# ANRGUSC/DEFER

Hardware: NVIDIA H100
Metric: inferences_per_sec (higher is better)
Workload: dtype bf16x3->f32

## Files before the change

defer_b200/csrc/conv_umma.cu:

```cuda
#include <cuda.h>
#include <string.h>

#include <type_traits>

#include <vector>

#include "common.cuh"
#include "conv_umma.cuh"

namespace defer {

static int env_int(const char* name, int dflt) {
  const char* v = getenv(name);
  return v ? atoi(v) : dflt;
}

namespace {

constexpr int BM = 128;
constexpr int BK = 64;
constexpr int CONS_THREADS = 256;
constexpr int NUM_THREADS = CONS_THREADS + 128;
constexpr int SMEM_CAP = 227 * 1024 - 256;
constexpr int CTL_BYTES = 256;
constexpr int MAX_STAGES = 8;
constexpr int MEGA_BN = 64;
constexpr int STG_COLS = 64;
constexpr int STG_BYTES = BM * STG_COLS * 4;

struct KParams {
  int n, ho, wo, cout;
  int tile_h, tile_w, tiles_h, tiles_w;
  int im2col;
  int m_total;
  int kh, kw, sh, sw, pad_t, pad_l;
  int cblocks;
  int k_blocks;
  int splits;
  int cluster;
  uint32_t flags;
  const float* scale;
  const float* shift;
  const void* res;
  void* y;
  float* partial;
  unsigned int* counters;
  size_t plane_out;
};

struct alignas(128) MegaOp {
  CUtensorMap tmx[2];
  CUtensorMap tmw[2];
  KParams p;
  int m_tiles, n_tiles;
  const float* stem_x;
  int stem_h, stem_w, stem_cin, stem_kh, stem_kw, stem_sh, stem_sw, stem_pad_t, stem_pad_l, stem_K;
  int stem_win_rows, stem_win_cols;
  const uint8_t* stem_u8;
  float stem_shift[3];
  const float* scale2;
  const float* shift2;
  void* y2;
  int relu2;
  int store_first;
};

template <int NPLANES, int BN>
struct Smem {
  static constexpr int A_PLANE = BM * 128;
  static constexpr int B_PLANE = BN * 128;
  static constexpr int STAGE = NPLANES * (A_PLANE + B_PLANE);
  static constexpr int RED = BM * BN * 4;
  __host__ __device__ static constexpr int ring(int stages, bool red) {
    return (red && stages * STAGE < RED) ? RED : stages * STAGE;
  }
  __host__ __device__ static constexpr int total(int stages, bool red) {
    return ring(stages, red) + STG_BYTES + CTL_BYTES + 1024;
  }
  __host__ __device__ static constexpr int max_stages() {
    return (SMEM_CAP - STG_BYTES - CTL_BYTES - 1024) / STAGE > MAX_STAGES ? MAX_STAGES
                                                                          : (SMEM_CAP - STG_BYTES - CTL_BYTES - 1024) / STAGE;
  }
};
static_assert(Smem<2, 128>::max_stages() == 3 && Smem<2, 64>::max_stages() == 4, "BF16X2 ring depths");
static_assert(Smem<1, 64>::max_stages() == 8 && Smem<1, 128>::max_stages() == 6, "BF16 ring depths");

__device__ __forceinline__ uint32_t smem_u32(const void* p) { return (uint32_t)__cvta_generic_to_shared(p); }

__device__ __forceinline__ void mbar_init(uint32_t bar, uint32_t count) {
  asm volatile("mbarrier.init.shared::cta.b64 [%0], %1;" ::"r"(bar), "r"(count));
}
__device__ __forceinline__ void mbar_arrive_expect_tx(uint32_t bar, uint32_t bytes) {
  asm volatile("mbarrier.arrive.expect_tx.shared::cta.b64 _, [%0], %1;" ::"r"(bar), "r"(bytes) : "memory");
}
__device__ __forceinline__ void mbar_expect_tx(uint32_t bar, uint32_t bytes) {
  asm volatile("mbarrier.expect_tx.relaxed.cta.shared::cta.b64 [%0], %1;" ::"r"(bar), "r"(bytes) : "memory");
}
__device__ __forceinline__ void mbar_arrive(uint32_t bar) {
  asm volatile("mbarrier.arrive.shared::cta.b64 _, [%0];" ::"r"(bar) : "memory");
}
__device__ __forceinline__ bool mbar_try_wait(uint32_t bar, uint32_t parity) {
  uint32_t ok;
  asm volatile(
      "{\n.reg .pred p;\n"
      "mbarrier.try_wait.parity.shared::cta.b64 p, [%1], %2;\n"
      "selp.u32 %0, 1, 0, p;\n}\n"
      : "=r"(ok)
      : "r"(bar), "r"(parity)
      : "memory");
  return ok != 0;
}
__device__ __forceinline__ unsigned long long gtimer() {
  unsigned long long t;
  asm volatile("mov.u64 %0, %%globaltimer;" : "=l"(t));
  return t;
}
__device__ int g_conv_wait_timeout_tag;
__device__ __forceinline__ void mbar_wait(uint32_t bar, uint32_t parity, int tag) {
  if (mbar_try_wait(bar, parity)) return;
  unsigned long long t0 = gtimer();
  unsigned spins = 0;
  while (!mbar_try_wait(bar, parity)) {
    if ((++spins & 0xfff) == 0 && gtimer() - t0 > 2000000000ull) {
      g_conv_wait_timeout_tag = tag;
      asm volatile("trap;");
    }
  }
}

__device__ __forceinline__ void tma_load_4d(uint32_t dst, const CUtensorMap* map, uint32_t bar, int c0, int c1, int c2,
                                            int c3) {
  asm volatile(
      "cp.async.bulk.tensor.4d.shared::cluster.global.mbarrier::complete_tx::bytes [%0], [%1, {%3, %4, %5, %6}], [%2];"
      ::"r"(dst), "l"(reinterpret_cast<uint64_t>(map)), "r"(bar), "r"(c0), "r"(c1), "r"(c2), "r"(c3)
      : "memory");
}
__device__ __forceinline__ void tma_load_im2col_4d(uint32_t dst, const CUtensorMap* map, uint32_t bar, int c0, int w, int h,
                                                   int n, uint16_t ow, uint16_t oh) {
  asm volatile(
      "cp.async.bulk.tensor.4d.shared::cluster.global.im2col.mbarrier::complete_tx::bytes [%0], [%1, {%3, %4, %5, %6}], "
      "[%2], {%7, %8};"
      ::"r"(dst), "l"(reinterpret_cast<uint64_t>(map)), "r"(bar), "r"(c0), "r"(w), "r"(h), "r"(n), "h"(ow), "h"(oh)
      : "memory");
}
__device__ __forceinline__ void tma_load_3d(uint32_t dst, const CUtensorMap* map, uint32_t bar, int c0, int c1, int c2) {
  asm volatile(
      "cp.async.bulk.tensor.3d.shared::cluster.global.mbarrier::complete_tx::bytes [%0], [%1, {%3, %4, %5}], [%2];"
      ::"r"(dst), "l"(reinterpret_cast<uint64_t>(map)), "r"(bar), "r"(c0), "r"(c1), "r"(c2)
      : "memory");
}

__device__ __forceinline__ void cluster_sync_all() {
  asm volatile("barrier.cluster.arrive.release.aligned;" ::: "memory");
  asm volatile("barrier.cluster.wait.acquire.aligned;" ::: "memory");
}
__device__ __forceinline__ uint32_t cluster_ctarank() {
  uint32_t r;
  asm volatile("mov.u32 %0, %%cluster_ctarank;" : "=r"(r));
  return r;
}
__device__ __forceinline__ uint32_t cluster_nctarank() {
  uint32_t r;
  asm volatile("mov.u32 %0, %%cluster_nctarank;" : "=r"(r));
  return r;
}
__device__ __forceinline__ uint32_t dsmem_map(uint32_t local_addr, uint32_t rank) {
  uint32_t r;
  asm volatile("mapa.shared::cluster.u32 %0, %1, %2;" : "=r"(r) : "r"(local_addr), "r"(rank));
  return r;
}
__device__ __forceinline__ float4 dsmem_ld4(uint32_t addr) {
  float4 v;
  asm volatile("ld.shared::cluster.v4.f32 {%0, %1, %2, %3}, [%4];" : "=f"(v.x), "=f"(v.y), "=f"(v.z), "=f"(v.w) : "r"(addr));
  return v;
}
__device__ __forceinline__ void cons_bar_sync() { asm volatile("bar.sync 1, 256;" ::: "memory"); }
__device__ __forceinline__ void prod_bar_sync() { asm volatile("bar.sync 2, 128;" ::: "memory"); }

__device__ __forceinline__ uint64_t make_sw128_desc(uint32_t smem_addr) {
  return (uint64_t)((smem_addr & 0x3FFFF) >> 4) | (1ull << 16) | (64ull << 32) | (1ull << 62);
}
__device__ __forceinline__ void wg_fence() { asm volatile("wgmma.fence.sync.aligned;" ::: "memory"); }
__device__ __forceinline__ void wg_commit() { asm volatile("wgmma.commit_group.sync.aligned;" ::: "memory"); }
template <int N>
__device__ __forceinline__ void wg_wait() {
  asm volatile("wgmma.wait_group.sync.aligned %0;" ::"n"(N) : "memory");
}
template <int R>
__device__ __forceinline__ void acc_fence(float (&d)[R]) {
#pragma unroll
  for (int i = 0; i < R; ++i) asm volatile("" : "+f"(d[i])::"memory");
}

template <int BN>
__device__ __forceinline__ void wgmma_bf16(float (&d)[BN / 2], uint64_t a, uint64_t b);

template <>
__device__ __forceinline__ void wgmma_bf16<64>(float (&d)[32], uint64_t a, uint64_t b) {
  asm volatile(
      "{\n.reg .pred p;\nsetp.ne.b32 p, %34, 0;\n"
      "wgmma.mma_async.sync.aligned.m64n64k16.f32.bf16.bf16 "
      "{%0, %1, %2, %3, %4, %5, %6, %7, %8, %9, %10, %11, %12, %13, %14, %15, %16, %17, %18, %19, %20, %21, %22, "
      "%23, %24, %25, %26, %27, %28, %29, %30, %31}, %32, %33, p, 1, 1, 0, 0;\n}\n"
      : "+f"(d[0]), "+f"(d[1]), "+f"(d[2]), "+f"(d[3]), "+f"(d[4]), "+f"(d[5]), "+f"(d[6]), "+f"(d[7]), "+f"(d[8]),
        "+f"(d[9]), "+f"(d[10]), "+f"(d[11]), "+f"(d[12]), "+f"(d[13]), "+f"(d[14]), "+f"(d[15]), "+f"(d[16]),
        "+f"(d[17]), "+f"(d[18]), "+f"(d[19]), "+f"(d[20]), "+f"(d[21]), "+f"(d[22]), "+f"(d[23]), "+f"(d[24]),
        "+f"(d[25]), "+f"(d[26]), "+f"(d[27]), "+f"(d[28]), "+f"(d[29]), "+f"(d[30]), "+f"(d[31])
      : "l"(a), "l"(b), "r"(1));
}

template <>
__device__ __forceinline__ void wgmma_bf16<128>(float (&d)[64], uint64_t a, uint64_t b) {
  asm volatile(
      "{\n.reg .pred p;\nsetp.ne.b32 p, %66, 0;\n"
      "wgmma.mma_async.sync.aligned.m64n128k16.f32.bf16.bf16 "
      "{%0, %1, %2, %3, %4, %5, %6, %7, %8, %9, %10, %11, %12, %13, %14, %15, %16, %17, %18, %19, %20, %21, %22, "
      "%23, %24, %25, %26, %27, %28, %29, %30, %31, %32, %33, %34, %35, %36, %37, %38, %39, %40, %41, %42, %43, %44, "
      "%45, %46, %47, %48, %49, %50, %51, %52, %53, %54, %55, %56, %57, %58, %59, %60, %61, %62, %63}, %64, %65, p, "
      "1, 1, 0, 0;\n}\n"
      : "+f"(d[0]), "+f"(d[1]), "+f"(d[2]), "+f"(d[3]), "+f"(d[4]), "+f"(d[5]), "+f"(d[6]), "+f"(d[7]), "+f"(d[8]),
        "+f"(d[9]), "+f"(d[10]), "+f"(d[11]), "+f"(d[12]), "+f"(d[13]), "+f"(d[14]), "+f"(d[15]), "+f"(d[16]),
        "+f"(d[17]), "+f"(d[18]), "+f"(d[19]), "+f"(d[20]), "+f"(d[21]), "+f"(d[22]), "+f"(d[23]), "+f"(d[24]),
        "+f"(d[25]), "+f"(d[26]), "+f"(d[27]), "+f"(d[28]), "+f"(d[29]), "+f"(d[30]), "+f"(d[31]), "+f"(d[32]),
        "+f"(d[33]), "+f"(d[34]), "+f"(d[35]), "+f"(d[36]), "+f"(d[37]), "+f"(d[38]), "+f"(d[39]), "+f"(d[40]),
        "+f"(d[41]), "+f"(d[42]), "+f"(d[43]), "+f"(d[44]), "+f"(d[45]), "+f"(d[46]), "+f"(d[47]), "+f"(d[48]),
        "+f"(d[49]), "+f"(d[50]), "+f"(d[51]), "+f"(d[52]), "+f"(d[53]), "+f"(d[54]), "+f"(d[55]), "+f"(d[56]),
        "+f"(d[57]), "+f"(d[58]), "+f"(d[59]), "+f"(d[60]), "+f"(d[61]), "+f"(d[62]), "+f"(d[63])
      : "l"(a), "l"(b), "r"(1));
}

template <bool STEM>
__device__ __forceinline__ void row_to_pixel(const KParams& p, int r, int n0, int h0, int w0, bool& valid, size_t& pix) {
  if (!STEM) {
    const int m = w0 + r;
    valid = m < p.m_total;
    pix = (size_t)m;
  } else {
    const int th = r / p.tile_w;
    const int oh = h0 + th, ow = w0 + r % p.tile_w;
    valid = th < p.tile_h && oh < p.ho && ow < p.wo;
    pix = ((size_t)n0 * p.ho + oh) * p.wo + ow;
  }
}

struct EpiArgs {
  const float* scale;
  const float* shift;
  const __nv_bfloat16* res;
  __nv_bfloat16* y;
  size_t plane;
  int cout;
  bool relu;
  bool store_first;
  bool relu2;
  const float* scale2;
  const float* shift2;
  __nv_bfloat16* y2;
};

__device__ __forceinline__ EpiArgs epi_args(const MegaOp& op) {
  const KParams& p = op.p;
  EpiArgs e;
  e.scale = p.scale;
  e.shift = p.shift;
  e.res = reinterpret_cast<const __nv_bfloat16*>(p.res);
  e.y = reinterpret_cast<__nv_bfloat16*>(p.y);
  e.plane = p.plane_out;
  e.cout = p.cout;
  e.relu = (p.flags & DEFER_FLAG_RELU) != 0;
  e.store_first = op.store_first != 0;
  e.relu2 = op.relu2 != 0;
  e.scale2 = op.scale2;
  e.shift2 = op.shift2;
  e.y2 = reinterpret_cast<__nv_bfloat16*>(op.y2);
  return e;
}

__device__ __forceinline__ uint32_t stg_off(int r, int c) {
  return (uint32_t)(r * STG_COLS + (((c >> 2) ^ ((r & 7) << 1)) << 2) + (c & 3)) * 4u;
}
__device__ __forceinline__ void sts2(uint32_t addr, float a, float b) {
  asm volatile("st.shared.v2.f32 [%0], {%1, %2};" ::"r"(addr), "f"(a), "f"(b));
}
__device__ __forceinline__ float4 lds4(uint32_t addr) {
  float4 v;
  asm volatile("ld.shared.v4.f32 {%0, %1, %2, %3}, [%4];" : "=f"(v.x), "=f"(v.y), "=f"(v.z), "=f"(v.w) : "r"(addr));
  return v;
}
__device__ __forceinline__ void stg4(void* p, uint4 v) {
  asm volatile("st.global.v4.b32 [%0], {%1, %2, %3, %4};" ::"l"(p), "r"(v.x), "r"(v.y), "r"(v.z), "r"(v.w));
}

__device__ __forceinline__ float bf_lo(uint32_t w) { return __uint_as_float(w << 16); }
__device__ __forceinline__ float bf_hi(uint32_t w) { return __uint_as_float(w & 0xffff0000u); }

template <int NPLANES, int BN, bool AFF, bool STEM = false>
__device__ __forceinline__ void epi_tile(const KParams& p, const EpiArgs& e, uint32_t stg, const float (&acc)[BN / 2],
                                         uint32_t qmask, int c_base, int n0, int h0, int w0) {
  const int tid = threadIdx.x;
  const int lane = tid & 31;
  const int row0 = (tid >> 7) * 64 + ((tid >> 5) & 3) * 16 + (lane >> 2);
  const int col_l = 2 * (lane & 3);
  const int jg = tid & 7;
  const int rb = tid >> 3;
  const int ca = 2 * jg + ((jg >> 2) & 1), cb = ca ^ 1;
  const bool swap = (jg >> 2) & 1;
  size_t orow[4];
  uint32_t vmask = 0;
#pragma unroll
  for (int k = 0; k < 4; ++k) {
    bool v;
    size_t pix;
    row_to_pixel<STEM>(p, rb + 32 * k, n0, h0, w0, v, pix);
    orow[k] = pix * (size_t)e.cout;
    vmask |= (uint32_t)v << k;
  }
#pragma unroll
  for (int P = 0; P < BN / STG_COLS; ++P) {
    const bool mine = (qmask >> (8 * P + jg)) & 1u;
    const int c = c_base + STG_COLS * P + 8 * jg;
    cons_bar_sync();
#pragma unroll
    for (int qq = 0; qq < 8; ++qq) {
      const int q = 8 * P + qq;
      if (!((qmask >> q) & 1u)) continue;
      sts2(stg + stg_off(row0, 8 * qq + col_l), acc[4 * q], acc[4 * q + 1]);
      sts2(stg + stg_off(row0 + 8, 8 * qq + col_l), acc[4 * q + 2], acc[4 * q + 3]);
    }
    uint4 rh[4], rl[4];
#pragma unroll
    for (int k = 0; k < 4; ++k) {
      rh[k] = rl[k] = make_uint4(0u, 0u, 0u, 0u);
      if (e.res && mine && ((vmask >> k) & 1u)) {
        rh[k] = __ldcg(reinterpret_cast<const uint4*>(e.res + orow[k] + c));
        if (NPLANES == 2) rl[k] = __ldcg(reinterpret_cast<const uint4*>(e.res + e.plane + orow[k] + c));
      }
    }
    float sc[8], sf[8];
#pragma unroll
    for (int i = 0; i < 8; ++i) { sc[i] = 1.f; sf[i] = 0.f; }
    if (mine) {
      if (e.scale) {
        const float4 a = __ldg(reinterpret_cast<const float4*>(e.scale + c));
        const float4 b = __ldg(reinterpret_cast<const float4*>(e.scale + c + 4));
        sc[0] = a.x; sc[1] = a.y; sc[2] = a.z; sc[3] = a.w; sc[4] = b.x; sc[5] = b.y; sc[6] = b.z; sc[7] = b.w;
      }
      if (e.shift) {
        const float4 a = __ldg(reinterpret_cast<const float4*>(e.shift + c));
        const float4 b = __ldg(reinterpret_cast<const float4*>(e.shift + c + 4));
        sf[0] = a.x; sf[1] = a.y; sf[2] = a.z; sf[3] = a.w; sf[4] = b.x; sf[5] = b.y; sf[6] = b.z; sf[7] = b.w;
      }
    }
    cons_bar_sync();
    if (!mine) continue;

#pragma unroll
    for (int k = 0; k < 4; ++k) {
      if (!((vmask >> k) & 1u)) continue;
      const int r = rb + 32 * k;
      const float4 xa = lds4(stg + stg_off(r, 4 * ca));
      const float4 xb = lds4(stg + stg_off(r, 4 * cb));
      const float4 x0 = swap ? xb : xa, x1 = swap ? xa : xb;
      float v[8] = {x0.x, x0.y, x0.z, x0.w, x1.x, x1.y, x1.z, x1.w};
      const uint32_t hw[4] = {rh[k].x, rh[k].y, rh[k].z, rh[k].w};
      const uint32_t lw[4] = {rl[k].x, rl[k].y, rl[k].z, rl[k].w};
#pragma unroll
      for (int i = 0; i < 8; ++i) {
        v[i] = fmaf(v[i], sc[i], sf[i]);
        if (e.res) {
          v[i] += (i & 1) ? bf_hi(hw[i >> 1]) : bf_lo(hw[i >> 1]);
          if (NPLANES == 2) v[i] += (i & 1) ? bf_hi(lw[i >> 1]) : bf_lo(lw[i >> 1]);
        }
        if (e.relu) v[i] = fmaxf(v[i], 0.f);
      }
      uint4 hi, lo = make_uint4(0u, 0u, 0u, 0u);
      if (NPLANES == 2) {
        split_bf16x2(v[0], v[1], hi.x, lo.x);
        split_bf16x2(v[2], v[3], hi.y, lo.y);
        split_bf16x2(v[4], v[5], hi.z, lo.z);
        split_bf16x2(v[6], v[7], hi.w, lo.w);
      } else {
        hi = make_uint4(pack_bf16x2(v[0], v[1]), pack_bf16x2(v[2], v[3]), pack_bf16x2(v[4], v[5]), pack_bf16x2(v[6], v[7]));
      }
      const size_t o = orow[k] + c;
      if (!AFF || e.store_first) {
        stg4(e.y + o, hi);
        if (NPLANES == 2) stg4(e.y + e.plane + o, lo);
      }
      if constexpr (AFF) {
        float s2[8], t2[8];
        {
          const float4 a = __ldg(reinterpret_cast<const float4*>(e.scale2 + c));
          const float4 b = __ldg(reinterpret_cast<const float4*>(e.scale2 + c + 4));
          const float4 d = __ldg(reinterpret_cast<const float4*>(e.shift2 + c));
          const float4 f = __ldg(reinterpret_cast<const float4*>(e.shift2 + c + 4));
          s2[0] = a.x; s2[1] = a.y; s2[2] = a.z; s2[3] = a.w; s2[4] = b.x; s2[5] = b.y; s2[6] = b.z; s2[7] = b.w;
          t2[0] = d.x; t2[1] = d.y; t2[2] = d.z; t2[3] = d.w; t2[4] = f.x; t2[5] = f.y; t2[6] = f.z; t2[7] = f.w;
        }
        const uint32_t sh[4] = {hi.x, hi.y, hi.z, hi.w};
        const uint32_t sl[4] = {lo.x, lo.y, lo.z, lo.w};
        float u[8];
#pragma unroll
        for (int i = 0; i < 8; ++i) {
          u[i] = (i & 1) ? bf_hi(sh[i >> 1]) : bf_lo(sh[i >> 1]);
          if (NPLANES == 2) u[i] = u[i] + ((i & 1) ? bf_hi(sl[i >> 1]) : bf_lo(sl[i >> 1]));
          u[i] = fmaf(u[i], s2[i], t2[i]);
          if (e.relu2) u[i] = fmaxf(u[i], 0.f);
        }
        uint4 h2, l2;
        if (NPLANES == 2) {
          split_bf16x2(u[0], u[1], h2.x, l2.x);
          split_bf16x2(u[2], u[3], h2.y, l2.y);
          split_bf16x2(u[4], u[5], h2.z, l2.z);
          split_bf16x2(u[6], u[7], h2.w, l2.w);
          stg4(e.y2 + o, h2);
          stg4(e.y2 + e.plane + o, l2);
        } else {
          h2 = make_uint4(pack_bf16x2(u[0], u[1]), pack_bf16x2(u[2], u[3]), pack_bf16x2(u[4], u[5]), pack_bf16x2(u[6], u[7]));
          stg4(e.y2 + o, h2);
        }
      }
    }
  }
}

template <int NPLANES, int BN, int MODE, bool AFF = false>
__device__ __forceinline__ void conv_body(const MegaOp* ops, int n_ops, int stages, int pdl) {
  using L = Smem<NPLANES, BN>;
  constexpr int R = BN / 2;
  extern __shared__ uint8_t smem_raw[];
  uint8_t* smem = reinterpret_cast<uint8_t*>((reinterpret_cast<uintptr_t>(smem_raw) + 1023) & ~(uintptr_t)1023);
  const uint32_t ring = smem_u32(smem);
  const bool red = MODE == 0 && ops[0].p.cluster;
  const uint32_t stg = ring + L::ring(stages, red);
  const uint32_t bar_base = stg + STG_BYTES;
  auto full_bar = [&](int s) { return bar_base + 8u * s; };
  auto empty_bar = [&](int s) { return bar_base + 8u * (stages + s); };
  __shared__ int s_is_last;

  const int tid = threadIdx.x;
  if (tid == 0) {
    for (int s = 0; s < stages; ++s) {
      mbar_init(full_bar(s), 1);
      mbar_init(empty_bar(s), CONS_THREADS / 32);
    }
    asm volatile("fence.mbarrier_init.release.cluster;" ::: "memory");
  }
  __syncthreads();
  if (pdl) {
    asm volatile("griddepcontrol.wait;" ::: "memory");
    asm volatile("griddepcontrol.launch_dependents;" ::: "memory");
  }

  uint32_t it = 0;
  for (int o = 0; o < n_ops; ++o) {
    const MegaOp& op = ops[o];
    const KParams& p = op.p;
    const int total = op.m_tiles * op.n_tiles;
    int t_first, t_step;
    if (MODE == 0) {
      t_first = blockIdx.y * op.m_tiles + blockIdx.x;
      t_step = total;
    } else if (MODE == 1) {
      t_first = blockIdx.x;
      t_step = gridDim.x;
    } else {
      t_first = (int)cluster_ctarank();
      t_step = (int)cluster_nctarank();
    }
    const int split = MODE == 0 ? (int)blockIdx.z : 0;
    const int kb_begin = (split * p.k_blocks) / p.splits;
    const int kb_end = ((split + 1) * p.k_blocks) / p.splits;

    for (int t = t_first; t < total; t += t_step) {
      const int m0 = (t % op.m_tiles) * BM;
      const int c_base = (t / op.m_tiles) * BN;

      if (tid >= CONS_THREADS) {
        if (tid == CONS_THREADS) {
          const int ow = m0 % p.wo;
          const int oh = (m0 / p.wo) % p.ho;
          const int cw = ow * p.sw - p.pad_l, ch = oh * p.sh - p.pad_t, cn = m0 / (p.wo * p.ho);
          uint32_t i2 = it;
          for (int kb = kb_begin; kb < kb_end; ++kb, ++i2) {
            const int stage = (int)(i2 % (uint32_t)stages);
            const uint32_t phase = (i2 / (uint32_t)stages) & 1u;
            mbar_wait(empty_bar(stage), phase ^ 1u, 1);
            const uint32_t a_dst = ring + stage * L::STAGE;
            const uint32_t b_dst = a_dst + NPLANES * L::A_PLANE;
            const int tap = kb / p.cblocks;
            const int cb = kb - tap * p.cblocks;
            const uint16_t khi = (uint16_t)(tap / p.kw);
            const uint16_t kwi = (uint16_t)(tap - khi * p.kw);
            mbar_arrive_expect_tx(full_bar(stage), NPLANES * (uint32_t)(L::A_PLANE + L::B_PLANE));
#pragma unroll
            for (int pl = 0; pl < NPLANES; ++pl) {
              if (p.im2col)
                tma_load_im2col_4d(a_dst + pl * L::A_PLANE, &op.tmx[pl], full_bar(stage), cb * BK, cw, ch, cn, kwi, khi);
              else
                tma_load_4d(a_dst + pl * L::A_PLANE, &op.tmx[pl], full_bar(stage), cb * BK, m0, 0, 0);
              tma_load_3d(b_dst + pl * L::B_PLANE, &op.tmw[pl], full_bar(stage), cb * BK, c_base, tap);
            }
          }
        }
        it += (uint32_t)(kb_end - kb_begin);
        continue;
      }

      const int wg = tid >> 7;
      const int lane = tid & 31;
      float acc[R];
#pragma unroll
      for (int i = 0; i < R; ++i) acc[i] = 0.f;
      int prev_stage = -1;
      for (int kb = kb_begin; kb < kb_end; ++kb, ++it) {
        const int stage = (int)(it % (uint32_t)stages);
        mbar_wait(full_bar(stage), (it / (uint32_t)stages) & 1u, 2);
        const uint32_t a_addr = ring + stage * L::STAGE + wg * (64 * 128);
        const uint32_t b_addr = ring + stage * L::STAGE + NPLANES * L::A_PLANE;
        wg_fence();
#pragma unroll
        for (int k = 0; k < BK / 16; ++k) {
          const uint64_t a_hi = make_sw128_desc(a_addr + k * 32);
          const uint64_t b_hi = make_sw128_desc(b_addr + k * 32);
          wgmma_bf16<BN>(acc, a_hi, b_hi);
          if (NPLANES == 2) {
            wgmma_bf16<BN>(acc, make_sw128_desc(a_addr + L::A_PLANE + k * 32), b_hi);
            wgmma_bf16<BN>(acc, a_hi, make_sw128_desc(b_addr + L::B_PLANE + k * 32));
          }
        }
        wg_commit();
        wg_wait<1>();
        acc_fence(acc);
        if (prev_stage >= 0 && lane == 0) mbar_arrive(empty_bar(prev_stage));
        prev_stage = stage;
      }
      wg_wait<0>();
      acc_fence(acc);
      if (prev_stage >= 0 && lane == 0) mbar_arrive(empty_bar(prev_stage));


      if (MODE == 0 && p.cluster) {
        cons_bar_sync();
        float4* red_buf = reinterpret_cast<float4*>(smem);
#pragma unroll
        for (int q = 0; q < R / 4; ++q)
          red_buf[q * CONS_THREADS + tid] = make_float4(acc[4 * q], acc[4 * q + 1], acc[4 * q + 2], acc[4 * q + 3]);
        break;
      }
      if (MODE == 0 && p.splits > 1) {
        const size_t tile_lin = (size_t)t;
        float4* mine = reinterpret_cast<float4*>(p.partial) + (tile_lin * p.splits + split) * (R / 4) * CONS_THREADS;
#pragma unroll
        for (int q = 0; q < R / 4; ++q)
          __stcg(mine + q * CONS_THREADS + tid, make_float4(acc[4 * q], acc[4 * q + 1], acc[4 * q + 2], acc[4 * q + 3]));
        __threadfence();
        cons_bar_sync();
        if (tid == 0) {
          const unsigned prev = atomicAdd(p.counters + tile_lin, 1u);
          const int last = prev == (unsigned)(p.splits - 1);
          if (last) p.counters[tile_lin] = 0;
          s_is_last = last;
        }
        cons_bar_sync();
        if (!s_is_last) continue;
        __threadfence();
#pragma unroll
        for (int i = 0; i < R; ++i) acc[i] = 0.f;
        for (int s = 0; s < p.splits; ++s) {
          const float4* src = reinterpret_cast<const float4*>(p.partial) + (tile_lin * p.splits + s) * (R / 4) * CONS_THREADS;
#pragma unroll
          for (int q = 0; q < R / 4; ++q) {
            const float4 v = __ldcg(src + q * CONS_THREADS + tid);
            acc[4 * q] += v.x; acc[4 * q + 1] += v.y; acc[4 * q + 2] += v.z; acc[4 * q + 3] += v.w;
          }
        }
      }
      epi_tile<NPLANES, BN, AFF>(p, epi_args(op), stg, acc, 0xffffu, c_base, 0, 0, m0);
    }

    if (MODE == 0 && p.cluster) {
      cluster_sync_all();
      if (tid < CONS_THREADS) {
        const int S = p.splits;
        const int rank = (int)cluster_ctarank();
        const uint32_t mine = ring + (uint32_t)tid * 16u;
        float acc[R];
        uint32_t qmask = 0;
#pragma unroll
        for (int q = 0; q < R / 4; ++q) {
          acc[4 * q] = acc[4 * q + 1] = acc[4 * q + 2] = acc[4 * q + 3] = 0.f;
          if (q % S != rank) continue;
          qmask |= 1u << q;
          const uint32_t addr = mine + (uint32_t)(q * CONS_THREADS) * 16u;
          float4 a = dsmem_ld4(dsmem_map(addr, 0));
          for (int s = 1; s < S; ++s) {
            const float4 v = dsmem_ld4(dsmem_map(addr, (uint32_t)s));
            a.x += v.x; a.y += v.y; a.z += v.z; a.w += v.w;
          }
          acc[4 * q] = a.x; acc[4 * q + 1] = a.y; acc[4 * q + 2] = a.z; acc[4 * q + 3] = a.w;
        }
        epi_tile<NPLANES, BN, AFF>(p, epi_args(op), stg, acc, qmask, (int)blockIdx.y * BN, 0, 0, (int)blockIdx.x * BM);
      }
      cluster_sync_all();
    }
    if (MODE == 2 && o + 1 < n_ops) {
      asm volatile("fence.proxy.async.global;" ::: "memory");
      cluster_sync_all();
    }
  }
}

template <int NPLANES, int BN>
__global__ void __launch_bounds__(NUM_THREADS, 1) conv_umma_kernel(const __grid_constant__ MegaOp op, int stages, int pdl) {
  conv_body<NPLANES, BN, 0>(&op, 1, stages, pdl);
}

template <int NPLANES, int BN>
__global__ void __launch_bounds__(NUM_THREADS, 1) conv_stream_kernel(const MegaOp* __restrict__ ops, int stages, int pdl) {
  conv_body<NPLANES, BN, 1>(ops, 1, stages, pdl);
}

template <int NPLANES, int BN>
__global__ void __launch_bounds__(NUM_THREADS, 1) conv_umma_aff_kernel(const __grid_constant__ MegaOp op, int stages, int pdl) {
  conv_body<NPLANES, BN, 0, true>(&op, 1, stages, pdl);
}

template <int NPLANES, int BN>
__global__ void __launch_bounds__(NUM_THREADS, 1) conv_stream_aff_kernel(const MegaOp* __restrict__ ops, int stages, int pdl) {
  conv_body<NPLANES, BN, 1, true>(ops, 1, stages, pdl);
}

template <int NPLANES>
__global__ void __launch_bounds__(NUM_THREADS, 1) conv_mega_kernel(const MegaOp* __restrict__ ops, int n_ops, int stages) {
  conv_body<NPLANES, MEGA_BN, 2>(ops, n_ops, stages, 0);
}

enum StemIn { STEM_F32, STEM_U8_CAFFE, STEM_U8_TF };
constexpr int PROD_THREADS = NUM_THREADS - CONS_THREADS;
constexpr int STEM_WIN_BYTES = 24 * 1024;
constexpr int STEM_WIN_VALS = STEM_WIN_BYTES / 4;
constexpr int STEM_FILL = STEM_WIN_VALS / PROD_THREADS;
constexpr int STEM_TILE_W = 16;

template <int NPLANES>
struct StemSmem {
  static constexpr int STAGE = Smem<NPLANES, 64>::STAGE;
  __host__ __device__ static constexpr int total(int stages) {
    return stages * STAGE + STG_BYTES + 2 * STEM_WIN_BYTES + CTL_BYTES + 1024;
  }
  __host__ __device__ static constexpr int max_stages() {
    return (SMEM_CAP - STG_BYTES - 2 * STEM_WIN_BYTES - CTL_BYTES - 1024) / STAGE > MAX_STAGES
               ? MAX_STAGES
               : (SMEM_CAP - STG_BYTES - 2 * STEM_WIN_BYTES - CTL_BYTES - 1024) / STAGE;
  }
};
static_assert(StemSmem<2>::max_stages() == 3 && StemSmem<1>::max_stages() == 6, "stem ring depths with two image windows");
static_assert(STEM_FILL * PROD_THREADS == STEM_WIN_VALS, "the producer threads cover a whole window");

struct StemGeo {
  const float* x;
  const uint8_t* u8;
  float s0, s1, s2;
  int H, rowlen;
  int cin, sh, sw, pad_t, pad_l;
  int wcols, nwin;
  int run, K;
};

__device__ __forceinline__ StemGeo stem_geo(const MegaOp& op) {
  StemGeo g;
  g.x = op.stem_x;
  g.u8 = op.stem_u8;
  g.s0 = op.stem_shift[0]; g.s1 = op.stem_shift[1]; g.s2 = op.stem_shift[2];
  g.H = op.stem_h;
  g.rowlen = op.stem_w * op.stem_cin;
  g.cin = op.stem_cin; g.sh = op.stem_sh; g.sw = op.stem_sw; g.pad_t = op.stem_pad_t; g.pad_l = op.stem_pad_l;
  g.wcols = op.stem_win_cols;
  g.nwin = op.stem_win_rows * op.stem_win_cols;
  g.run = op.stem_kw * op.stem_cin;
  g.K = op.stem_K;
  return g;
}

__device__ __forceinline__ void stem_tile_origin(const KParams& p, int m_tile, int& n0, int& h0, int& w0) {
  const int t2 = m_tile / p.tiles_w;
  n0 = t2 / p.tiles_h;
  h0 = (t2 - n0 * p.tiles_h) * p.tile_h;
  w0 = (m_tile - t2 * p.tiles_w) * p.tile_w;
}

template <int IN>
__device__ __forceinline__ void stem_fill_load(const StemGeo& g, int ptid, int n0, int h0, int w0, uint32_t (&raw)[STEM_FILL]) {
  const int ih0 = h0 * g.sh - g.pad_t, col0 = (w0 * g.sw - g.pad_l) * g.cin;
  const size_t img = (size_t)n0 * g.H * g.rowlen;
  const int dq = PROD_THREADS / g.wcols, dm = PROD_THREADS - dq * g.wcols;
  int wr = ptid / g.wcols, wc = ptid - wr * g.wcols;
  int c = wc % 3;
#pragma unroll
  for (int j = 0; j < STEM_FILL; ++j) {
    const int ih = ih0 + wr, col = col0 + wc;
    const bool in = ptid + PROD_THREADS * j < g.nwin && ih >= 0 && ih < g.H && col >= 0 && col < g.rowlen;
    const size_t off = img + (size_t)(ih * g.rowlen + col);
    if constexpr (IN == STEM_F32) raw[j] = in ? __float_as_uint(__ldg(g.x + off)) : 0u;
    else raw[j] = in ? (uint32_t)__ldg(g.u8 + off + (IN == STEM_U8_CAFFE ? 2 - 2 * c : 0)) : 0x100u;
    wr += dq;
    wc += dm;
    if (wc >= g.wcols) { wc -= g.wcols; ++wr; }
    c = c == 0 ? 2 : c - 1;
  }
}

template <int IN>
__device__ __forceinline__ void stem_fill_store(const StemGeo& g, uint32_t win, int ptid, const uint32_t (&raw)[STEM_FILL]) {
  int c = (ptid % g.wcols) % 3;
#pragma unroll
  for (int j = 0; j < STEM_FILL; ++j) {
    const int e = ptid + PROD_THREADS * j;
    if (e < g.nwin) {
      const float b = __fsub_rn(__uint_as_float(0x4B000000u | raw[j]), 8388608.f);
      float v;
      if constexpr (IN == STEM_F32) v = __uint_as_float(raw[j]);
      else if constexpr (IN == STEM_U8_CAFFE) v = raw[j] > 255u ? 0.f : __fadd_rn(b, c == 0 ? g.s0 : (c == 1 ? g.s1 : g.s2));
      else v = raw[j] > 255u ? 0.f : keras_tf_preprocess(b);
      asm volatile("st.shared.f32 [%0], %1;" ::"r"(win + 4u * (uint32_t)e), "f"(v) : "memory");
    }
    c = c == 0 ? 2 : c - 1;
  }
}

template <int NPLANES>
__device__ __forceinline__ void stem_build(const StemGeo& g, uint32_t win, uint32_t a_dst, int r, int row_base, int kb) {
  int k = kb * BK;
  int a = k / g.run, jj = k - a * g.run;
  uint32_t src = win + 4u * (uint32_t)(row_base + a * g.wcols + jj);
  const uint32_t wrap = 4u * (uint32_t)(g.wcols - g.run);
#pragma unroll 1
  for (int ch = 0; ch < 8; ++ch) {
    float v[8];
#pragma unroll
    for (int e = 0; e < 8; ++e) {
      v[e] = 0.f;
      if (k < g.K) asm volatile("ld.shared.f32 %0, [%1];" : "=f"(v[e]) : "r"(src));
      ++k;
      src += 4u;
      if (++jj == g.run) { jj = 0; src += wrap; }
    }
    const uint32_t off = (uint32_t)r * 128u + ((uint32_t)(ch ^ (r & 7)) << 4);
    uint32_t h[4], l[4];
#pragma unroll
    for (int q = 0; q < 4; ++q) {
      if (NPLANES == 2) split_bf16x2(v[2 * q], v[2 * q + 1], h[q], l[q]);
      else h[q] = pack_bf16x2(v[2 * q], v[2 * q + 1]);
    }
    asm volatile("st.shared.v4.b32 [%0], {%1, %2, %3, %4};" ::"r"(a_dst + off), "r"(h[0]), "r"(h[1]), "r"(h[2]), "r"(h[3])
                 : "memory");
    if (NPLANES == 2)
      asm volatile("st.shared.v4.b32 [%0], {%1, %2, %3, %4};" ::"r"(a_dst + Smem<NPLANES, 64>::A_PLANE + off), "r"(l[0]),
                   "r"(l[1]), "r"(l[2]), "r"(l[3])
                   : "memory");
  }
}

template <int NPLANES, int IN>
__device__ __forceinline__ void stem_body(const MegaOp* ops, int stages, int pdl) {
  using L = Smem<NPLANES, 64>;
  extern __shared__ uint8_t smem_raw[];
  uint8_t* smem = reinterpret_cast<uint8_t*>((reinterpret_cast<uintptr_t>(smem_raw) + 1023) & ~(uintptr_t)1023);
  const uint32_t ring = smem_u32(smem);
  const uint32_t stg = ring + stages * L::STAGE;
  const uint32_t win0 = stg + STG_BYTES;
  const uint32_t bar_base = win0 + 2 * STEM_WIN_BYTES;
  auto full_bar = [&](int s) { return bar_base + 8u * s; };
  auto empty_bar = [&](int s) { return bar_base + 8u * (stages + s); };

  const int tid = threadIdx.x;
  if (tid == 0) {
    for (int s = 0; s < stages; ++s) {
      mbar_init(full_bar(s), 1);
      mbar_init(empty_bar(s), CONS_THREADS / 32);
    }
    asm volatile("fence.mbarrier_init.release.cluster;" ::: "memory");
  }
  __syncthreads();
  if (pdl) {
    asm volatile("griddepcontrol.wait;" ::: "memory");
    asm volatile("griddepcontrol.launch_dependents;" ::: "memory");
  }

  const MegaOp& op = ops[0];
  const KParams& p = op.p;
  const int total = op.m_tiles * op.n_tiles;
  const int k_blocks = p.k_blocks;
  uint32_t it = 0;

  if (tid >= CONS_THREADS) {
    const int ptid = tid - CONS_THREADS;
    const StemGeo g = stem_geo(op);
    int th = ptid / p.tile_w, tw = ptid - th * p.tile_w;
    if (th >= p.tile_h) th = tw = 0;
    const int row_base = th * g.sh * g.wcols + tw * g.sw * g.cin;
    uint32_t raw[STEM_FILL];
    int n0, h0, w0;
    if ((int)blockIdx.x < total) {
      stem_tile_origin(p, (int)blockIdx.x % op.m_tiles, n0, h0, w0);
      stem_fill_load<IN>(g, ptid, n0, h0, w0, raw);
      stem_fill_store<IN>(g, win0, ptid, raw);
    }
    int wb = 0;
    for (int t = blockIdx.x; t < total; t += gridDim.x, wb ^= 1) {
      const int t_next = t + (int)gridDim.x;
      if (t_next < total) {
        stem_tile_origin(p, t_next % op.m_tiles, n0, h0, w0);
        stem_fill_load<IN>(g, ptid, n0, h0, w0, raw);
      }
      prod_bar_sync();
      const uint32_t win = win0 + (uint32_t)wb * STEM_WIN_BYTES;
      const int c_base = (t / op.m_tiles) * 64;
      for (int kb = 0; kb < k_blocks; ++kb, ++it) {
        const int stage = (int)(it % (uint32_t)stages);
        mbar_wait(empty_bar(stage), ((it / (uint32_t)stages) & 1u) ^ 1u, 1);
        const uint32_t a_dst = ring + stage * L::STAGE;
        const uint32_t b_dst = a_dst + NPLANES * L::A_PLANE;
        if (ptid == 0) {
          mbar_expect_tx(full_bar(stage), NPLANES * (uint32_t)L::B_PLANE);
          tma_load_3d(b_dst, &op.tmw[0], full_bar(stage), kb * BK, c_base, 0);
          if (NPLANES == 2) tma_load_3d(b_dst + L::B_PLANE, &op.tmw[1], full_bar(stage), kb * BK, c_base, 0);
        }
        stem_build<NPLANES>(g, win, a_dst, ptid, row_base, kb);
        asm volatile("fence.proxy.async.shared::cta;" ::: "memory");
        prod_bar_sync();
        if (ptid == 0) mbar_arrive(full_bar(stage));
      }
      if (t_next < total) stem_fill_store<IN>(g, win0 + (uint32_t)(wb ^ 1) * STEM_WIN_BYTES, ptid, raw);
    }
    return;
  }

  const int wg = tid >> 7;
  const int lane = tid & 31;
  for (int t = blockIdx.x; t < total; t += gridDim.x) {
    float acc[32];
#pragma unroll
    for (int i = 0; i < 32; ++i) acc[i] = 0.f;
    int prev_stage = -1;
    for (int kb = 0; kb < k_blocks; ++kb, ++it) {
      const int stage = (int)(it % (uint32_t)stages);
      mbar_wait(full_bar(stage), (it / (uint32_t)stages) & 1u, 2);
      const uint32_t a_addr = ring + stage * L::STAGE + wg * (64 * 128);
      const uint32_t b_addr = ring + stage * L::STAGE + NPLANES * L::A_PLANE;
      wg_fence();
#pragma unroll
      for (int k = 0; k < BK / 16; ++k) {
        const uint64_t a_hi = make_sw128_desc(a_addr + k * 32);
        const uint64_t b_hi = make_sw128_desc(b_addr + k * 32);
        wgmma_bf16<64>(acc, a_hi, b_hi);
        if (NPLANES == 2) {
          wgmma_bf16<64>(acc, make_sw128_desc(a_addr + L::A_PLANE + k * 32), b_hi);
          wgmma_bf16<64>(acc, a_hi, make_sw128_desc(b_addr + L::B_PLANE + k * 32));
        }
      }
      wg_commit();
      wg_wait<1>();
      acc_fence(acc);
      if (prev_stage >= 0 && lane == 0) mbar_arrive(empty_bar(prev_stage));
      prev_stage = stage;
    }
    wg_wait<0>();
    acc_fence(acc);
    if (prev_stage >= 0 && lane == 0) mbar_arrive(empty_bar(prev_stage));
    int n0, h0, w0;
    stem_tile_origin(p, t % op.m_tiles, n0, h0, w0);
    epi_tile<NPLANES, 64, false, true>(p, epi_args(op), stg, acc, 0xffffu, (t / op.m_tiles) * 64, n0, h0, w0);
  }
}

template <int NPLANES>
__global__ void __launch_bounds__(NUM_THREADS, 1) conv_stem_kernel(const MegaOp* __restrict__ ops, int stages, int pdl) {
  stem_body<NPLANES, STEM_F32>(ops, stages, pdl);
}

template <int NPLANES>
__global__ void __launch_bounds__(NUM_THREADS, 1) conv_stem_u8_kernel(const MegaOp* __restrict__ ops, int stages, int pdl) {
  stem_body<NPLANES, STEM_U8_CAFFE>(ops, stages, pdl);
}

template <int NPLANES>
__global__ void __launch_bounds__(NUM_THREADS, 1) conv_stem_u8tf_kernel(const MegaOp* __restrict__ ops, int stages, int pdl) {
  stem_body<NPLANES, STEM_U8_TF>(ops, stages, pdl);
}

__global__ void __launch_bounds__(256) weight_transform_kernel(const float* __restrict__ w, __nv_bfloat16* __restrict__ out,
                                                               int taps, int cin, int cout, int nplanes) {
  size_t total = (size_t)taps * cin * cout;
  size_t i = (size_t)blockIdx.x * blockDim.x + threadIdx.x;
  if (i >= total) return;
  int ci = (int)(i % cin);
  size_t t2 = i / cin;
  int co = (int)(t2 % cout);
  int tap = (int)(t2 / cout);
  float v = w[((size_t)tap * cin + ci) * cout + co];
  __nv_bfloat16 hi = __float2bfloat16_rn(v);
  out[i] = hi;
  if (nplanes == 2) out[total + i] = __float2bfloat16_rn(v - __bfloat162float(hi));
}

typedef CUresult (*PFN_encodeTiled)(CUtensorMap*, CUtensorMapDataType, cuuint32_t, void*, const cuuint64_t*,
                                    const cuuint64_t*, const cuuint32_t*, const cuuint32_t*, CUtensorMapInterleave,
                                    CUtensorMapSwizzle, CUtensorMapL2promotion, CUtensorMapFloatOOBfill);

PFN_encodeTiled get_encode() {
  static PFN_encodeTiled fn = nullptr;
  if (!fn) {
    void* p = nullptr;
    cudaDriverEntryPointQueryResult q;
    if (cudaGetDriverEntryPoint("cuTensorMapEncodeTiled", &p, cudaEnableDefault, &q) == cudaSuccess &&
        q == cudaDriverEntryPointSuccess)
      fn = (PFN_encodeTiled)p;
  }
  return fn;
}

int encode_map(CUtensorMap* map, void* base, int rank, const uint64_t* dims, const uint64_t* strides_bytes,
               const uint32_t* box, const uint32_t* estr) {
  PFN_encodeTiled enc = get_encode();
  if (!enc) {
    set_error("cuTensorMapEncodeTiled entry point not available");
    return DEFER_ERR_CUDA;
  }
  CUresult r = enc(map, CU_TENSOR_MAP_DATA_TYPE_BFLOAT16, (cuuint32_t)rank, base, (const cuuint64_t*)dims,
                   (const cuuint64_t*)strides_bytes, (const cuuint32_t*)box, (const cuuint32_t*)estr,
                   CU_TENSOR_MAP_INTERLEAVE_NONE, CU_TENSOR_MAP_SWIZZLE_128B, CU_TENSOR_MAP_L2_PROMOTION_L2_256B,
                   CU_TENSOR_MAP_FLOAT_OOB_FILL_NONE);
// ... 503 lines not shown
```

Before: 15370.

## Add dedicated warp-specialized stream kernel body with residual prefetch before mainloop

New measurement: 13820 (median of 6 runs). -10.1%, worse.

```diff
diff --git a/defer_b200/csrc/conv_umma.cu b/defer_b200/csrc/conv_umma.cu
--- a/defer_b200/csrc/conv_umma.cu
+++ b/defer_b200/csrc/conv_umma.cu
@@ -294,9 +294,10 @@
 __device__ __forceinline__ float bf_lo(uint32_t w) { return __uint_as_float(w << 16); }
 __device__ __forceinline__ float bf_hi(uint32_t w) { return __uint_as_float(w & 0xffff0000u); }
 
-template <int NPLANES, int BN, bool AFF, bool STEM = false>
+template <int NPLANES, int BN, bool AFF, bool STEM = false, bool PRE = false>
 __device__ __forceinline__ void epi_tile(const KParams& p, const EpiArgs& e, uint32_t stg, const float (&acc)[BN / 2],
-                                         uint32_t qmask, int c_base, int n0, int h0, int w0) {
+                                         uint32_t qmask, int c_base, int n0, int h0, int w0,
+                                         const uint4 (*pre)[2][4] = nullptr) {
   const int tid = threadIdx.x;
   const int lane = tid & 31;
   const int row0 = (tid >> 7) * 64 + ((tid >> 5) & 3) * 16 + (lane >> 2);
@@ -330,6 +331,11 @@
     uint4 rh[4], rl[4];
 #pragma unroll
     for (int k = 0; k < 4; ++k) {
+      if constexpr (PRE) {
+        rh[k] = pre[P][0][k];
+        rl[k] = pre[P][1][k];
+        continue;
+      }
       rh[k] = rl[k] = make_uint4(0u, 0u, 0u, 0u);
       if (e.res && mine && ((vmask >> k) & 1u)) {
         rh[k] = __ldcg(reinterpret_cast<const uint4*>(e.res + orow[k] + c));
@@ -424,6 +430,27 @@
   }
 }
 
+template <int NPLANES, int BN>
+__device__ __forceinline__ void epi_res_prefetch(const KParams& p, const EpiArgs& e, int c_base, int m0,
+                                                 uint4 (&pre)[BN / STG_COLS][2][4]) {
+  const int tid = threadIdx.x;
+  const int c = c_base + 8 * (tid & 7);
+  const int rb = tid >> 3;
+#pragma unroll
+  for (int P = 0; P < BN / STG_COLS; ++P) {
+#pragma unroll
+    for (int k = 0; k < 4; ++k) {
+      const int m = m0 + rb + 32 * k;
+      pre[P][0][k] = pre[P][1][k] = make_uint4(0u, 0u, 0u, 0u);
+      if (e.res && m < p.m_total) {
+        const size_t o = (size_t)m * (size_t)e.cout + (size_t)(c + STG_COLS * P);
+        pre[P][0][k] = __ldcg(reinterpret_cast<const uint4*>(e.res + o));
+        if (NPLANES == 2) pre[P][1][k] = __ldcg(reinterpret_cast<const uint4*>(e.res + e.plane + o));
+      }
+    }
+  }
+}
+
 template <int NPLANES, int BN, int MODE, bool AFF = false>
 __device__ __forceinline__ void conv_body(const MegaOp* ops, int n_ops, int stages, int pdl) {
   using L = Smem<NPLANES, BN>;
@@ -461,9 +488,6 @@
     if (MODE == 0) {
       t_first = blockIdx.y * op.m_tiles + blockIdx.x;
       t_step = total;
-    } else if (MODE == 1) {
-      t_first = blockIdx.x;
-      t_step = gridDim.x;
     } else {
       t_first = (int)cluster_ctarank();
       t_step = (int)cluster_nctarank();
@@ -611,6 +635,115 @@
   }
 }
 
+template <int NPLANES, int BN, bool AFF>
+__device__ __forceinline__ void stream_body(const MegaOp* ops, int stages, int pdl) {
+  using L = Smem<NPLANES, BN>;
+  constexpr int R = BN / 2;
+  extern __shared__ uint8_t smem_raw[];
+  uint8_t* smem = reinterpret_cast<uint8_t*>((reinterpret_cast<uintptr_t>(smem_raw) + 1023) & ~(uintptr_t)1023);
+  const uint32_t ring = smem_u32(smem);
+  const uint32_t stg = ring + L::ring(stages, false);
+  const uint32_t bar_base = stg + STG_BYTES;
+  auto full_bar = [&](int s) { return bar_base + 8u * s; };
+  auto empty_bar = [&](int s) { return bar_base + 8u * (stages + s); };
+
+  const int tid = threadIdx.x;
+  if (tid == 0) {
+    for (int s = 0; s < stages; ++s) {
+      mbar_init(full_bar(s), 1);
+      mbar_init(empty_bar(s), CONS_THREADS / 32);
+    }
+    asm volatile("fence.mbarrier_init.release.cluster;" ::: "memory");
+  }
+  __syncthreads();
+  if (pdl) {
+    asm volatile("griddepcontrol.wait;" ::: "memory");
+    asm volatile("griddepcontrol.launch_dependents;" ::: "memory");
+  }
+
+  const MegaOp& op = ops[0];
+  const KParams& p = op.p;
+
+  if (tid >= CONS_THREADS) {
+    asm volatile("setmaxnreg.dec.sync.aligned.u32 40;" ::: "memory");
+    if (tid != CONS_THREADS) return;
+    const int total = op.m_tiles * op.n_tiles;
+    const int k_blocks = p.k_blocks;
+    uint32_t it = 0;
+    for (int t = blockIdx.x; t < total; t += gridDim.x) {
+      const int m0 = (t % op.m_tiles) * BM;
+      const int c_base = (t / op.m_tiles) * BN;
+      const int ow = m0 % p.wo;
+      const int oh = (m0 / p.wo) % p.ho;
+      const int cw = ow * p.sw - p.pad_l, ch = oh * p.sh - p.pad_t, cn = m0 / (p.wo * p.ho);
+      for (int kb = 0; kb < k_blocks; ++kb, ++it) {
+        const int stage = (int)(it % (uint32_t)stages);
+        mbar_wait(empty_bar(stage), ((it / (uint32_t)stages) & 1u) ^ 1u, 1);
+        const uint32_t a_dst = ring + stage * L::STAGE;
+        const uint32_t b_dst = a_dst + NPLANES * L::A_PLANE;
+        const int tap = kb / p.cblocks;
+        const int cb = kb - tap * p.cblocks;
+        const uint16_t khi = (uint16_t)(tap / p.kw);
+        const uint16_t kwi = (uint16_t)(tap - khi * p.kw);
+        mbar_arrive_expect_tx(full_bar(stage), NPLANES * (uint32_t)(L::A_PLANE + L::B_PLANE));
+#pragma unroll
+        for (int pl = 0; pl < NPLANES; ++pl) {
+          if (p.im2col)
+            tma_load_im2col_4d(a_dst + pl * L::A_PLANE, &op.tmx[pl], full_bar(stage), cb * BK, cw, ch, cn, kwi, khi);
+          else
+            tma_load_4d(a_dst + pl * L::A_PLANE, &op.tmx[pl], full_bar(stage), cb * BK, m0, 0, 0);
+          tma_load_3d(b_dst + pl * L::B_PLANE, &op.tmw[pl], full_bar(stage), cb * BK, c_base, tap);
+        }
+      }
+    }
+    return;
+  }
+
+  asm volatile("setmaxnreg.inc.sync.aligned.u32 232;" ::: "memory");
+  const int total = op.m_tiles * op.n_tiles;
+  const int k_blocks = p.k_blocks;
+  const int wg = tid >> 7;
+  const int lane = tid & 31;
+  uint32_t it = 0;
+  for (int t = blockIdx.x; t < total; t += gridDim.x) {
+    const int m0 = (t % op.m_tiles) * BM;
+    const int c_base = (t / op.m_tiles) * BN;
+    uint4 pre[BN / STG_COLS][2][4];
+    epi_res_prefetch<NPLANES, BN>(p, epi_args(op), c_base, m0, pre);
+
+    float acc[R];
+#pragma unroll
+    for (int i = 0; i < R; ++i) acc[i] = 0.f;
+    int prev_stage = -1;
+    for (int kb = 0; kb < k_blocks; ++kb, ++it) {
+      const int stage = (int)(it % (uint32_t)stages);
+      mbar_wait(full_bar(stage), (it / (uint32_t)stages) & 1u, 2);
+      const uint32_t a_addr = ring + stage * L::STAGE + wg * (64 * 128);
+      const uint32_t b_addr = ring + stage * L::STAGE + NPLANES * L::A_PLANE;
+      wg_fence();
+#pragma unroll
+      for (int k = 0; k < BK / 16; ++k) {
+        const uint64_t a_hi = make_sw128_desc(a_addr + k * 32);
+        const uint64_t b_hi = make_sw128_desc(b_addr + k * 32);
+        wgmma_bf16<BN>(acc, a_hi, b_hi);
+        if (NPLANES == 2) {
+          wgmma_bf16<BN>(acc, make_sw128_desc(a_addr + L::A_PLANE + k * 32), b_hi);
+          wgmma_bf16<BN>(acc, a_hi, make_sw128_desc(b_addr + L::B_PLANE + k * 32));
+        }
+      }
+      wg_commit();
+      wg_wait<1>();
+      acc_fence(acc);
+      if (prev_stage >= 0 && lane == 0) mbar_arrive(empty_bar(prev_stage));
+      prev_stage = stage;
+    }
+    wg_wait<0>();
+    acc_fence(acc);
+    if (lane == 0) mbar_arrive(empty_bar(prev_stage));
+    epi_tile<NPLANES, BN, AFF, false, true>(p, epi_args(op), stg, acc, 0xffffu, c_base, 0, 0, m0, pre);
+  }
+}
+
 template <int NPLANES, int BN>
 __global__ void __launch_bounds__(NUM_THREADS, 1) conv_umma_kernel(const __grid_constant__ MegaOp op, int stages, int pdl) {
   conv_body<NPLANES, BN, 0>(&op, 1, stages, pdl);
@@ -618,7 +751,7 @@
 
 template <int NPLANES, int BN>
 __global__ void __launch_bounds__(NUM_THREADS, 1) conv_stream_kernel(const MegaOp* __restrict__ ops, int stages, int pdl) {
-  conv_body<NPLANES, BN, 1>(ops, 1, stages, pdl);
+  stream_body<NPLANES, BN, false>(ops, stages, pdl);
 }
 
 template <int NPLANES, int BN>
@@ -628,7 +761,7 @@
 
 template <int NPLANES, int BN>
 __global__ void __launch_bounds__(NUM_THREADS, 1) conv_stream_aff_kernel(const MegaOp* __restrict__ ops, int stages, int pdl) {
-  conv_body<NPLANES, BN, 1, true>(ops, 1, stages, pdl);
+  stream_body<NPLANES, BN, true>(ops, stages, pdl);
 }
 
 template <int NPLANES>
```
